# Wionerlol/MultimodalEmotionRecognition

Hardware: AMD Instinct MI355X
Metric: 3s-clip train steps/sec (B=32, xattn fusion) at 1/2/4/8 MI355X (higher is better)
Workload: dtype bf16; 1 GPU; ResNet18 + WavLM-base (frozen) + xattn fusion train step (fwd+bwd+Adam); per_gpu_batch=32, global_batch=32, frames=8, image=112, audio_samples=48000, parallelism=dp1

## Files before the change

### multimodalemotionrecognition_amd/csrc/conv.hip

```cpp
#include "conv_common.h"
#include "mer.h"

MER_CT_BUFFER(mer_ct, 512 * 64)
MER_CT_BUFFER(mer_ctp, 4096 * 8)
#define CT(k) CT_AT(mer_ct_buf, k)
#define CTP(k) CTP_AT(mer_ctp_buf, k)

namespace {

template <bool DGRAD>
__device__ __forceinline__ u32x4 conv_a_chunk(const ConvGeom& g, int n, int oh, int ow, bool rowok, int kk, int tap,
                                              int c, int r, int s) {
  u32x4 v = {0u, 0u, 0u, 0u};
  if (!rowok || kk >= g.Kred) return v;
  int ih, iw;
  if (!DGRAD) {
    ih = oh * g.st - g.pad + r;
    iw = ow * g.st - g.pad + s;
  } else {
    const int th = oh + g.pad - r, tw = ow + g.pad - s;
    if (th < 0 || tw < 0) return v;
    if (g.st == 1) {
      ih = th;
      iw = tw;
// ... 848 lines not shown
        const int kk = k0 + bcl[j];
        const bool ok = bok[j] && kk < Kr;
        const bf16_t* src = !PAR ? pb[j] + kk : (kk >= Kr0 ? pb2[j] + (kk - Kr0) : pb[j] + par_b_off(kk));
        glds16(ok ? src : zero, lb + (w * IB + j) * 512);
      }
      k0 += KS;
    });
  }
  CTP(2);

  auto out_row = [&](int row) -> long {
    if (!PAR) return (long)row;
    const int n = row / (pc.Hc * pc.Wc);
    const int rem = row - n * pc.Hc * pc.Wc;
    const int hh = rem / pc.Wc, ww = rem - hh * pc.Wc;
    return ((long)n * g.OH + 2 * hh + pc.ph) * g.OW + 2 * ww + pc.pw;
  };
  auto red_row = [&]() -> long {
    long row_id = ty;
    if (PAR)
      for (int c2 = 0; c2 < par_cls(); ++c2) {
        const ParClass q = par_class(g, c2);
        row_id += (g.N * q.Hc * q.Wc + BM_ - 1) / BM_;
      }
    return row_id;
  };
  constexpr int EWF = STAGES * BUF / 2 / WAVES;
  const int ct_slot = 10;
  if constexpr (KG > 1) {
    using L = KgLayout<BM_, BN_, WAVES * KG>;
    constexpr int LDR = BN_ + 4;
    constexpr int TM2 = BM_ / L::WM, TN2 = BN_ / L::WN, FM2 = TM2 / 16, FN2 = TN2 / 16;
    using E2 = EpiGeo<FM2, FN2, EWF>;
    const int w2 = t >> 6, wr2 = w2 / L::WN, wc2 = w2 % L::WN;
    constexpr bool PF = DGRAD && E2::NP == 1;
    EpiPre<E2::NP> pre;
    if constexpr (PF)
      conv_epilogue_prefetch<DGRAD, FM2, FN2, L::WM, L::WN, EWF, decltype(out_row), E2::NP, X2>(g, pre, w2, lane, m0,
                                                                                                n0, M, out_row);
    __syncthreads();
    float* const part = reinterpret_cast<float*>(smem_all);
    {
      float* mine = part + kg * BM_ * LDR;
#pragma unroll
      for (int i = 0; i < FM; ++i)
#pragma unroll
        for (int j = 0; j < FN; ++j)
#pragma unroll
          for (int r = 0; r < 4; ++r) mine[(wr * TM + i * 16 + fq * 4 + r) * LDR + wc * TN + j * 16 + fr] = acc[i][j][r];
    }
    lds_barrier();
    f32x4 acc2[FM2][FN2];
#pragma unroll
    for (int i = 0; i < FM2; ++i)
#pragma unroll
      for (int j = 0; j < FN2; ++j)
#pragma unroll
        for (int r = 0; r < 4; ++r) {
          const int e = (wr2 * TM2 + i * 16 + fq * 4 + r) * LDR + wc2 * TN2 + j * 16 + fr;
          float s = part[e];
#pragma unroll
          for (int q = 1; q < KG; ++q) s += part[q * BM_ * LDR + e];
          acc2[i][j][r] = s;
        }
    lds_barrier();
    CTP(3);
    if constexpr (PF)
      conv_epilogue_vec<DGRAD, FM2, FN2, L::WM, L::WN, EWF, decltype(out_row), decltype(pre), false, X2>(
          g, acc2, reinterpret_cast<float*>(smem_all), w2, lane, m0, n0, M, g.bnr_red ? red_row() : 0l, ty, out_row,
          &pre, ct_slot);
    else
      conv_epilogue_vec<DGRAD, FM2, FN2, L::WM, L::WN, EWF, decltype(out_row), EpiNone, false, X2>(
          g, acc2, reinterpret_cast<float*>(smem_all), w2, lane, m0, n0, M, (DGRAD && g.bnr_red) ? red_row() : 0l, ty,
          out_row, static_cast<const EpiNone*>(nullptr), ct_slot);
    CTP(4);
    return;
  }
  if (g.vec) {
    using E1 = EpiGeo<FM, FN, EWF>;
    if constexpr (DGRAD && E1::NP == 1) {
      EpiPre<E1::NP> pre;
      conv_epilogue_prefetch<DGRAD, FM, FN, WM, WN, EWF, decltype(out_row), E1::NP, X2>(g, pre, w, lane, m0, n0, M,
                                                                                         out_row);
      __syncthreads();
      CTP(3);
      conv_epilogue_vec<DGRAD, FM, FN, WM, WN, EWF, decltype(out_row), decltype(pre), false, X2>(
          g, acc, reinterpret_cast<float*>(smem), w, lane, m0, n0, M, g.bnr_red ? red_row() : 0l, ty, out_row, &pre,
          ct_slot);
    } else {
      __syncthreads();
      CTP(3);
      conv_epilogue_vec<DGRAD, FM, FN, WM, WN, EWF, decltype(out_row), EpiNone, false, X2>(
          g, acc, reinterpret_cast<float*>(smem), w, lane, m0, n0, M, (DGRAD && g.bnr_red) ? red_row() : 0l, ty,
          out_row, static_cast<const EpiNone*>(nullptr), ct_slot);
    }
    CTP(4);
    return;
  } else {
  __syncthreads();
#pragma unroll
  for (int i = 0; i < FM; ++i)
#pragma unroll
    for (int r = 0; r < 4; ++r) {
      const int row = m0 + wr * TM + i * 16 + fq * 4 + r;
      if (row >= M) continue;
      const long orow = out_row(row) * g.ldy;
#pragma unroll
      for (int j = 0; j < FN; ++j) {
        const int col = n0 + wc * TN + j * 16 + fr;
        if (col >= g.Ncols) continue;
        float v = acc[i][j][r];
        if (g.R_) {
          const long ri = orow + col;
          if (!g.Rmask || bf2f(g.Rmask[ri]) > 0.f) v += bf2f(g.R_[ri]);
        }
        const bf16_t h = f2bf(v);
        g.Y[orow + col] = h;
        acc[i][j][r] = bf2f(h);
      }
    }
  if (DGRAD && g.bnr_red) {
    float ps[FN][3];
#pragma unroll
    for (int j = 0; j < FN; ++j) {
      const int col = n0 + wc * TN + j * 16 + fr;
      const bool cok = col < g.Ncols;
      const float mu = cok ? g.bnr_ms[2 * col] : 0.f, rs = cok ? g.bnr_ms[2 * col + 1] : 0.f;
      const float mu2 = (cok && g.bnr_x2) ? g.bnr_ms2[2 * col] : 0.f;
      const float rs2 = (cok && g.bnr_x2) ? g.bnr_ms2[2 * col + 1] : 0.f;
      float s1 = 0.f, s2 = 0.f, s3 = 0.f;
#pragma unroll
      for (int i = 0; i < FM; ++i)
#pragma unroll
        for (int r = 0; r < 4; ++r) {
          const int row = m0 + wr * TM + i * 16 + fq * 4 + r;
          if (row < M && cok) {
            const long e = out_row(row) * g.ldy + col;
            const float gv = bf2f(g.bnr_mask[e]) > 0.f ? acc[i][j][r] : 0.f;
            s1 += gv;
            s2 += gv * (bf2f(g.bnr_x[e]) - mu) * rs;
            if (g.bnr_x2) s3 += gv * (bf2f(g.bnr_x2[e]) - mu2) * rs2;
          }
        }
#pragma unroll
      for (int o = 16; o < 64; o <<= 1) {
        s1 += __shfl_xor(s1, o, 64);
        s2 += __shfl_xor(s2, o, 64);
        s3 += __shfl_xor(s3, o, 64);
      }
      ps[j][0] = s1;
      ps[j][1] = s2;
      ps[j][2] = s3;
    }
    float* red = reinterpret_cast<float*>(smem);
    __syncthreads();
    if (wr > 0 && fq == 0)
#pragma unroll
      for (int j = 0; j < FN; ++j)
#pragma unroll
        for (int q = 0; q < 3; ++q) red[((wr * WN + wc) * FN * 16 + j * 16 + fr) * 3 + q] = ps[j][q];
    __syncthreads();
    if (wr == 0 && fq == 0) {
      long row_id = ty;
      if (PAR)
        for (int c2 = 0; c2 < par_cls(); ++c2) {
          const ParClass q = par_class(g, c2);
          row_id += (g.N * q.Hc * q.Wc + BM_ - 1) / BM_;
        }
      const long slab = row_id * g.Ncols * 2;
#pragma unroll
      for (int j = 0; j < FN; ++j) {
        const int col = n0 + wc * TN + j * 16 + fr;
        float t0 = ps[j][0], t1 = ps[j][1], t2 = ps[j][2];
#pragma unroll
        for (int q = 1; q < WM; ++q) {
          const float* o = red + ((q * WN + wc) * FN * 16 + j * 16 + fr) * 3;
          t0 += o[0];
          t1 += o[1];
          t2 += o[2];
        }
        if (col < g.Ncols) {
          g.bnr_red[slab + 2 * col] = t0;
          g.bnr_red[slab + 2 * col + 1] = t1;
          if (g.bnr_red2) {
            g.bnr_red2[slab + 2 * col] = t0;
            g.bnr_red2[slab + 2 * col + 1] = t2;
          }
        }
      }
    }
  }
  }
  if (g.stats) conv_tile_stats<FM, FN, WM, WN>(g, acc, reinterpret_cast<float*>(smem), w, lane, m0, n0, M, ty);
}

template <int BM_, int BN_, int WM_ = 2, int WN_ = 2, int STAGES_ = 2, int KS_ = 64, int KG_ = 1>
struct Tile {
  static constexpr int BM = BM_, BN = BN_, WM = WM_, WN = WN_, STAGES = STAGES_, KS = KS_, KG = KG_;
};

enum ConvFamily { kConvNone, kConvHalo, kConvReg, kConvPipe };

struct ConvPlan {
  int err;
  ConvFamily family;
  int halo;
  int variant;
  bool par;
  int BM, BN, WM, WN, STAGES, KS, KG;
  bool x2, fast;
  size_t lds;
  unsigned grid_x, grid_y;
  int rows;
};

template <bool DGRAD, bool PAR, class T>
int launch_conv_pipe_t(ConvGeom& g, const ConvPlan& p, hipStream_t st) {
  if (T::BM != p.BM || T::BN != p.BN || T::WM != p.WM || T::WN != p.WN || T::STAGES != p.STAGES || T::KS != p.KS ||
      T::KG != p.KG)
    return (int)hipErrorInvalidConfiguration;
  auto launch = [&](void (*kern)(ConvGeom)) -> int {
    if (hipFuncSetAttribute(reinterpret_cast<const void*>(kern), hipFuncAttributeMaxDynamicSharedMemorySize,
                            (int)p.lds) != hipSuccess)
      return (int)hipErrorInvalidConfiguration;
    hipLaunchKernelGGL(kern, dim3(p.grid_x, p.grid_y), dim3(64 * T::WM * T::WN * T::KG), p.lds, st, g);
    return (int)hipGetLastError();
  };
  if constexpr (DGRAD && !PAR) {
    if (!p.x2)
      return p.fast ? launch(&conv_pipe_kernel<DGRAD, PAR, T::BM, T::BN, T::WM, T::WN, T::STAGES, T::KS, false, T::KG,
                                               true>)
                    : launch(&conv_pipe_kernel<DGRAD, PAR, T::BM, T::BN, T::WM, T::WN, T::STAGES, T::KS, false, T::KG,
                                               false>);
  }
  return p.fast
             ? launch(&conv_pipe_kernel<DGRAD, PAR, T::BM, T::BN, T::WM, T::WN, T::STAGES, T::KS, true, T::KG, true>)
             : launch(&conv_pipe_kernel<DGRAD, PAR, T::BM, T::BN, T::WM, T::WN, T::STAGES, T::KS, true, T::KG, false>);
}

inline int conv_bn(const ConvGeom& g) { return g.Ncols <= 64 ? 64 : 128; }
inline bool conv_small_m(const ConvGeom& g, bool par) {
  const long M = (long)g.N * g.OH * g.OW / (par ? 4 : 1);
  const int bn = conv_bn(g);
  return ((M + 127) / 128) * ((g.Ncols + bn - 1) / bn) * (par ? 4 : 1) < 384;
}

template <bool DGRAD, bool PAR, class F>
int conv_pipe_tile(const ConvGeom& g, int variant, F&& f) {
  const int bn = conv_bn(g);
  const bool small_m = conv_small_m(g, PAR);
  if (variant == 7) {
    if (bn == 64) return PAR ? f(Tile<64, 64, 2, 2, 2, 64, 2>{}) : f(Tile<64, 64, 2, 2, 3, 64, 2>{});
    return PAR ? f(Tile<64, 128, 2, 4, 2, 64, 2>{}) : f(Tile<64, 128, 2, 4, 3, 64, 2>{});
  }
  if (variant == 3 && !small_m) {
    if constexpr (DGRAD) {
      return f(Tile<256, 64, 4, 2>{});
    } else {
      if (bn == 64) return f(Tile<256, 64, 4, 2>{});
      return f(Tile<256, 128, 4, 4>{});
    }
  }
  if (variant == 5) {
    if (bn == 64) return small_m ? f(Tile<64, 64, 2, 2, 4, 32>{}) : f(Tile<128, 64, 2, 2, 4, 32>{});
    return small_m ? f(Tile<64, 128, 2, 2, 4, 32>{}) : f(Tile<128, 128, 2, 4, 4, 32>{});
  }
  if (variant == 4) {
    if (bn == 64) return small_m ? f(Tile<64, 64, 2, 2, 3>{}) : f(Tile<128, 64, 4, 2, 3>{});
    return small_m ? f(Tile<64, 128, 2, 4, 3>{}) : f(Tile<128, 128, 2, 4, 3>{});
  }
  if (variant >= 2) {
    if (bn == 64)
      return small_m ? (PAR ? f(Tile<64, 64, 2, 2>{}) : f(Tile<64, 64, 2, 2, 3>{})) : f(Tile<128, 64, 4, 2>{});
    return small_m ? (PAR ? f(Tile<64, 128, 2, 4>{}) : f(Tile<64, 128, 2, 4, 3>{})) : f(Tile<128, 128, 2, 4>{});
  }
  if (bn == 64) return small_m ? f(Tile<64, 64>{}) : f(Tile<128, 64>{});
  return small_m ? f(Tile<64, 128>{}) : f(Tile<128, 128>{});
}

template <bool DGRAD>
int launch_conv(ConvGeom& g, const ConvPlan& p, hipStream_t st) {
  auto launch = [&](void (*kern)(ConvGeom)) -> int {
    hipLaunchKernelGGL(kern, dim3(p.grid_x), dim3(256), 0, st, g);
    return (int)hipGetLastError();
  };
  if (p.BN == 64) return p.BM == 64 ? launch(&conv_kernel<DGRAD, 64, 64>) : launch(&conv_kernel<DGRAD, 128, 64>);
  return p.BM == 64 ? launch(&conv_kernel<DGRAD, 64, 128>) : launch(&conv_kernel<DGRAD, 128, 128>);
}

namespace halo {
constexpr int BM = 128;
template <int C_, int R_, int PAD_, int W_, int IHX_>
struct Geo {
  static constexpr int C = C_, R = R_, PAD = PAD_, W = W_, IHX = IHX_;
  static constexpr int KRED = R * R * C, WCH = KRED / 8;
  static constexpr int CPP = C / 8;
  static constexpr int HW = W + R - 1;
  static constexpr int ROWS = (W + BM - 2) / W + 1 + (R - 1) + IHX;
  static constexpr int CH = (ROWS * HW * CPP + 63) / 64 * 64;
  static constexpr int ELEMS = CH * 8;
  static constexpr int LDS_ELEMS = 64 * KRED + 2 * ELEMS + C;
  static constexpr int KSTEPS = KRED / 32;
  static constexpr int HSHIFT = CPP == 8 ? 1 : 3;
  static_assert(CPP == 8 || CPP == 2, "halo layouts for 16 or 64 channels");
  static_assert(WCH % 16 == 0 || WCH % 16 == 8, "weight-row swizzle");
};
template <int WCH>
__device__ __forceinline__ int wchunk(int n, int c) {
  return WCH % 16 == 0 ? ((c & ~15) | ((c & 15) ^ (n & 15))) : ((c & ~7) | ((c & 7) ^ ((n >> 1) & 7)));
}
}

template <bool DGRAD, class GE, int WM, int WN, int OCC, bool X2 = true>
__global__ __launch_bounds__(64 * WM * WN, OCC) void conv_halo_kernel(ConvGeom g) {
  constexpr int WAVES = WM * WN;
  constexpr int TM = halo::BM / WM, TN = 64 / WN, FM = TM / 16, FN = TN / 16;
  constexpr int HW = GE::HW, CPP = GE::CPP, C = GE::C, R = GE::R, PAD = GE::PAD, W_ = GE::W;
  extern __shared__ __attribute__((aligned(16))) bf16_t smem[];
  bf16_t* const wlds = smem;
  bf16_t* const hbuf = smem + 64 * GE::KRED;
  bf16_t* const zpix = hbuf + 2 * GE::ELEMS;
  const int t = threadIdx.x, lane = t & 63, w = t >> 6;
  const int wr = w / WN, wc = w % WN, fr = lane & 15, fq = lane >> 4;
  const int OH = g.OH, IH = g.IH, IW = g.IW, M = g.N * g.OH * W_, in_rows = g.N * g.IH;
  const int ntiles = (M + halo::BM - 1) / halo::BM;
  const bf16_t* zero = reinterpret_cast<const bf16_t*>(mer_conv_zero16);
  int tile = blockIdx.x;
  CT(0);
  auto in_row0 = [&](int m) {
    const int go = m / W_, n = go / OH;
    return n * IH + (go - n * OH) - PAD;
  };
  auto stage_halo = [&](bf16_t* hb, int tl) {
    const int base = in_row0(tl * halo::BM);
    for (int j = w; j < GE::CH / 64; j += WAVES) {
      const int L = j * 64 + lane;
      const int hp = L / CPP, c = (L % CPP) ^ ((hp >> GE::HSHIFT) & (CPP - 1));
      const int hr = hp / HW, x = hp - hr * HW - PAD, gr = base + hr;
      const bool ok = hr < GE::ROWS && gr >= 0 && gr < in_rows && x >= 0 && x < IW;
      glds16(ok ? g.X + ((long)gr * IW + x) * C + c * 8 : zero, hb + j * 512);
    }
  };
  for (int j = w; j < GE::WCH; j += WAVES) {
    const int L = j * 64 + lane;
    const int n = L / GE::WCH, pc = L - n * GE::WCH;
    glds16(g.Wt + (long)n * GE::KRED + halo::wchunk<GE::WCH>(n, pc) * 8, wlds + j * 512);
  }
  stage_halo(hbuf, tile);
  if (t < CPP) *reinterpret_cast<u32x4*>(zpix + t * 8) = u32x4{0u, 0u, 0u, 0u};
  wait_vmcnt<0>();
  __syncthreads();
  CT(1);

  EpiAcc<FN> eacc;
  eacc.zero();
  for (int cur = 0, it = 0; tile < ntiles; tile += gridDim.x, cur ^= 1, ++it) {
    bf16_t* const hb = hbuf + cur * GE::ELEMS;
    if (tile + (int)gridDim.x < ntiles) stage_halo(hbuf + (cur ^ 1) * GE::ELEMS, tile + gridDim.x);
    CT(it < 11 ? 2 + 5 * it : 63);
    const int m0 = tile * halo::BM, base = in_row0(m0);
    const auto out_row = [](int row) { return (long)row; };
    constexpr int EWF = GE::ELEMS / 2 / WAVES;
    EpiPre<EpiGeo<FM, FN, EWF>::NP> pre;
    if constexpr (DGRAD)
      conv_epilogue_prefetch<DGRAD, FM, FN, WM, WN, EWF, decltype(out_row), EpiGeo<FM, FN, EWF>::NP, X2>(
          g, pre, w, lane, m0, 0, M, out_row);
    int hpb[FM], yv[FM];
#pragma unroll
    for (int i = 0; i < FM; ++i) {
      int m = m0 + wr * TM + i * 16 + fr;
      m = m < M ? m : M - 1;
      const int go = m / W_, x = m - go * W_, n = go / OH, y = go - n * OH;
      yv[i] = y - PAD;
      hpb[i] = (n * IH + y - PAD - base) * HW + x;
    }
    f32x4 acc[FM][FN];
#pragma unroll
    for (int i = 0; i < FM; ++i)
#pragma unroll
      for (int j = 0; j < FN; ++j) acc[i][j] = f32x4{0.f, 0.f, 0.f, 0.f};
    bf16x8 af[2][FM], bfr[2][FN];
    auto frags = [&](int u, bf16x8 (&a)[FM], bf16x8 (&b)[FN]) {
      const int kk = u * 32 + fq * 8;
      const int tap = kk / C, c = (kk % C) / 8;
      const int r = tap / R, s = tap - R * (tap / R);
      const int hr = DGRAD ? R - 1 - r : r, hs = DGRAD ? R - 1 - s : s;
#pragma unroll
      for (int i = 0; i < FM; ++i) {
        const int hp = hpb[i] + hr * HW + hs;
        const bool ok = (unsigned)(yv[i] + hr) < (unsigned)IH;
        a[i] = *reinterpret_cast<const bf16x8*>(
            ok ? hb + hp * C + ((c ^ ((hp >> GE::HSHIFT) & (CPP - 1))) << 3) : zpix);
      }
#pragma unroll
      for (int j = 0; j < FN; ++j) {
        const int n = wc * TN + j * 16 + fr, cb = u * 4 + fq;
        b[j] = *reinterpret_cast<const bf16x8*>(wlds + n * GE::KRED + (halo::wchunk<GE::WCH>(n, cb) << 3));
      }
    };
    frags(0, af[0], bfr[0]);
#pragma unroll
    for (int u = 0; u < GE::KSTEPS; ++u) {
      if (u + 1 < GE::KSTEPS) frags(u + 1, af[(u + 1) & 1], bfr[(u + 1) & 1]);
#pragma unroll
      for (int i = 0; i < FM; ++i)
#pragma unroll
        for (int j = 0; j < FN; ++j)
          acc[i][j] = __builtin_amdgcn_mfma_f32_16x16x32_bf16(af[u & 1][i], bfr[u & 1][j], acc[i][j], 0, 0, 0);
    }
    CT(it < 11 ? 3 + 5 * it : 63);
    wait_vmcnt<0>();
    lds_barrier();
    CT(it < 11 ? 4 + 5 * it : 63);
    const int ct_slot = it == 1 ? 60 : -1;
    if constexpr (DGRAD)
      conv_epilogue_vec<DGRAD, FM, FN, WM, WN, EWF, decltype(out_row), decltype(pre), true, X2, EpiAcc<FN>>(
          g, acc, reinterpret_cast<float*>(hb), w, lane, m0, 0, M, (long)tile, (long)tile, out_row, &pre, ct_slot,
          &eacc);
    else
      conv_epilogue_vec<DGRAD, FM, FN, WM, WN, EWF, decltype(out_row), EpiNone, true, true, EpiAcc<FN>>(
          g, acc, reinterpret_cast<float*>(hb), w, lane, m0, 0, M, (long)tile, (long)tile, out_row,
          static_cast<const EpiNone*>(nullptr), ct_slot, &eacc);
    CT(it < 11 ? 5 + 5 * it : 63);
    lds_barrier();
    CT(it < 11 ? 6 + 5 * it : 63);
  }
  conv_epilogue_acc_finish<DGRAD, FM, FN, WM, WN, GE::ELEMS / 2 / WAVES, X2>(g, eacc, reinterpret_cast<float*>(hbuf), w,
                                                                          lane, 0, (long)blockIdx.x);
}

using HaloL1 = halo::Geo<64, 3, 1, 28, 0>;
using HaloStem = halo::Geo<16, 4, 0, 56, 3>;

int halo_kind(const ConvGeom& g, bool dgrad) {
  if (g.st != 1 || g.Ncols != 64 || g.ldy != 64 || !g.vec || g.X2 != nullptr ||
      ((((uintptr_t)g.X) | ((uintptr_t)g.Wt)) & 15) != 0)
    return 0;
  if (g.R == 3 && g.S == 3 && g.pad == 1 && g.IC == 64 && g.IW == 28 && g.OW == 28 && g.IH == g.OH && g.Kred == 576)
    return 1;
  if (!dgrad && g.R == 4 && g.S == 4 && g.pad == 0 && g.IC == 16 && g.IW == 59 && g.OW == 56 && g.IH == 59 &&
      g.OH == 56 && g.Kred == 256)
    return 2;
  return 0;
}

template <bool DGRAD, class GE, int OCC, bool X2 = true>
int launch_halo_t(ConvGeom& g, const ConvPlan& p, hipStream_t st) {
  constexpr int WM = 4, WN = 2;
  const size_t lds = GE::LDS_ELEMS * sizeof(bf16_t);
  static_assert(GE::LDS_ELEMS * 2 * OCC <= 160 * 1024, "LDS per CU");
  if (hipFuncSetAttribute(reinterpret_cast<const void*>(&conv_halo_kernel<DGRAD, GE, WM, WN, OCC, X2>),
                          hipFuncAttributeMaxDynamicSharedMemorySize, (int)lds) != hipSuccess)
    return (int)hipErrorInvalidConfiguration;
  hipLaunchKernelGGL((conv_halo_kernel<DGRAD, GE, WM, WN, OCC, X2>), dim3(p.grid_x), dim3(64 * WM * WN), lds, st, g);
  return (int)hipGetLastError();
}

constexpr int halo_occ(int kind) { return kind == 1 ? 1 : 2; }

template <bool DGRAD>
int launch_conv_halo(ConvGeom& g, const ConvPlan& p, hipStream_t st) {
  if constexpr (DGRAD)
    if (p.halo == 1 && !p.x2) return launch_halo_t<DGRAD, HaloL1, halo_occ(1), false>(g, p, st);
  if (p.halo == 1) return launch_halo_t<DGRAD, HaloL1, halo_occ(1)>(g, p, st);
  if constexpr (!DGRAD) return launch_halo_t<false, HaloStem, halo_occ(2)>(g, p, st);
  return (int)hipErrorInvalidValue;
}

int conv_default_variant(const ConvGeom& g, int fallback) {
  if (!g.vec || g.Kred < 8 * CBK) return fallback;
  const long M = (long)g.N * g.OH * g.OW;
  const long nt = (g.Ncols + (g.Ncols <= 64 ? 63 : 127)) / (g.Ncols <= 64 ? 64 : 128);
  if (((M + 63) / 64) * nt <= cu_count()) return 7;
  return fallback;
}

template <class F>
int conv_pipe_tile_of(const ConvGeom& g, bool dgrad, bool par, int variant, F&& f) {
  if (!dgrad) return conv_pipe_tile<false, false>(g, variant, f);
  return par ? conv_pipe_tile<true, true>(g, variant, f) : conv_pipe_tile<true, false>(g, variant, f);
}

ConvPlan conv_plan(const ConvGeom& g, bool dgrad, int variant) {
  ConvPlan p{};
  const long M = (long)g.N * g.OH * g.OW;
  const long nx = (g.Ncols + conv_bn(g) - 1) / conv_bn(g);
  p.grid_y = 1;
  p.x2 = true;
  if (variant == -1 || variant == 6) {
    if (const int hk = halo_kind(g, dgrad)) {
      const long ntiles = (M + halo::BM - 1) / halo::BM, slots = (long)halo_occ(hk) * cu_count();
      p.family = kConvHalo;
      p.halo = hk;
      p.variant = 6;
      p.BM = halo::BM; p.BN = 64; p.WM = 4; p.WN = 2;
      p.x2 = !(dgrad && hk == 1 && !g.bnr_x2);
      p.grid_x = (unsigned)(ntiles < slots ? ntiles : slots);
      p.rows = (int)p.grid_x;
      return p;
    }
    if (variant == 6) {
      p.err = (int)hipErrorInvalidValue;
      return p;
    }
    variant = dgrad ? (g.Ncols <= 64 ? 5 : 2) : 2;
    if (!dgrad || g.st == 1) variant = conv_default_variant(g, variant);
  }
  p.variant = variant;
  if (variant == 0 || (dgrad && g.st > 2)) {
    p.family = kConvReg;
    p.BM = conv_small_m(g, false) ? 64 : 128;
    p.BN = conv_bn(g);
    p.WM = p.WN = 2;
    p.rows = (int)((M + p.BM - 1) / p.BM);
    p.grid_x = (unsigned)(nx * p.rows);
    return p;
  }
  p.family = kConvPipe;
  p.par = dgrad && g.st == 2;
  conv_pipe_tile_of(g, dgrad, p.par, variant, [&](auto t) {
    using T = decltype(t);
    p.BM = T::BM; p.BN = T::BN; p.WM = T::WM; p.WN = T::WN; p.STAGES = T::STAGES; p.KS = T::KS; p.KG = T::KG;
    return 0;
  });
  if (p.KG > 1 && !g.vec) p.err = (int)hipErrorInvalidValue;
  const size_t ring = (size_t)p.KG * p.STAGES * (p.BM + p.BN) * p.KS * sizeof(bf16_t);
  const size_t kgred = p.KG > 1 ? (size_t)p.KG * p.BM * (p.BN + 4) * sizeof(float) : 0;
  p.lds = ring > kgred ? ring : kgred;
  p.x2 = !(dgrad && !p.par && !g.bnr_x2);
  p.fast = p.par ? (g.IC % p.KS == 0 && (!g.X2 || g.K2 % p.KS == 0) && ((g.R + 1) / 2) * ((g.S + 1) / 2) <= 32)
                 : (g.IC % p.KS == 0 && g.R * g.S <= 32 && (!dgrad || g.st == 1));
  const long nbn = (g.Ncols + p.BN - 1) / p.BN;
  if (!p.par) {
    p.rows = (int)((M + p.BM - 1) / p.BM);
    p.grid_x = (unsigned)(p.rows * nbn);
    return p;
  }
  p.grid_y = 4;
  for (int cls = 0; cls < 4; ++cls) {
    const int ph = cls >> 1, pw = cls & 1;
    const long Mc = (long)g.N * ((g.OH - ph + 1) >> 1) * ((g.OW - pw + 1) >> 1);
    p.rows += (int)((Mc + p.BM - 1) / p.BM);
    if (cls == 0) p.grid_x = (unsigned)((Mc + p.BM - 1) / p.BM * nbn);
  }
  return p;
}

template <bool DGRAD>
int launch_conv_plan(ConvGeom& g, const ConvPlan& p, hipStream_t st) {
  if (p.err != (int)hipSuccess) return p.err;
  if (p.family == kConvHalo) return launch_conv_halo<DGRAD>(g, p, st);
  if (p.family == kConvReg) return launch_conv<DGRAD>(g, p, st);
  if constexpr (DGRAD)
    if (p.par)
      return conv_pipe_tile<true, true>(g, p.variant,
                                        [&](auto t) { return launch_conv_pipe_t<true, true, decltype(t)>(g, p, st); });
  return conv_pipe_tile<DGRAD, false>(g, p.variant,
                                      [&](auto t) { return launch_conv_pipe_t<DGRAD, false, decltype(t)>(g, p, st); });
}

int conv_plan_rows(const ConvGeom& g, bool dgrad, int variant) {
  const ConvPlan p = conv_plan(g, dgrad, variant);
  if (p.family == kConvHalo || (variant == -1 && p.family == kConvPipe)) return p.rows;
  return (int)(((long)g.N * g.OH * g.OW + 63) / 64 + (dgrad ? 4 : 0));
}

ConvGeom fwd_geom(int N, int H, int W, int C, int K, int R, int S, int stride, int pad, const void* x,
                  const void* w_packed, void* y, float* stats) {
  ConvGeom g{};
  g.N = N; g.IH = H; g.IW = W; g.IC = C;
  g.OH = (H + 2 * pad - R) / stride + 1; g.OW = (W + 2 * pad - S) / stride + 1;
  g.R = R; g.S = S; g.st = stride; g.pad = pad;
  g.Ncols = K; g.Kred = R * S * C;
  g.X = (const bf16_t*)x; g.Wt = (const bf16_t*)w_packed; g.Y = (bf16_t*)y; g.ldy = K; g.stats = stats;
  g.vec = conv_vec_ok(g);
  return g;
}

ConvGeom dgrad_geom(int N, int H, int W, int C, int K, int R, int S, int stride, int pad, const void* dy,
                    const void* wt_packed, const void* ds_dy) {
  ConvGeom g{};
  g.N = N; g.OH = H; g.OW = W;
  g.IH = (H + 2 * pad - R) / stride + 1; g.IW = (W + 2 * pad - S) / stride + 1; g.IC = K;
  g.R = R; g.S = S; g.st = stride; g.pad = pad;
  g.Ncols = C; g.Kred = R * S * K;
  g.X = (const bf16_t*)dy; g.Wt = (const bf16_t*)wt_packed; g.ldy = C; g.stats = nullptr;
  g.X2 = (const bf16_t*)ds_dy;
  g.vec = conv_vec_ok(g);
  return g;
}

}

MER_API int mer_conv_fwd(int N, int H, int W, int C, int K, int R, int S, int stride, int pad, const void* x,
                         const void* w_packed, void* y, float* stats, void* stream) {
  return mer_conv_fwd_ex(N, H, W, C, K, R, S, stride, pad, x, w_packed, y, stats, -1, stream);
}

MER_API int mer_conv_fwd_rows(int N, int H, int W, int C, int K, int R, int S, int stride, int pad, const void* x,
                              const void* w_packed, int variant) {
  if (N <= 0 || C % 8 || variant < -1 || variant > 7) return -(int)hipErrorInvalidValue;
  return conv_plan_rows(fwd_geom(N, H, W, C, K, R, S, stride, pad, x, w_packed, nullptr, nullptr), false, variant);
}

MER_API int mer_conv_dgrad_rows(int N, int H, int W, int C, int K, int R, int S, int stride, int pad, const void* dy,
                                const void* wt_packed, const void* ds_dy, int variant) {
  if (N <= 0 || K % 8 || C % 8 || variant < -1 || variant > 7) return -(int)hipErrorInvalidValue;
  return conv_plan_rows(dgrad_geom(N, H, W, C, K, R, S, stride, pad, dy, wt_packed, ds_dy), true, variant);
}

MER_API int mer_conv_fwd_ex(int N, int H, int W, int C, int K, int R, int S, int stride, int pad, const void* x,
                            const void* w_packed, void* y, float* stats, int variant, void* stream) {
  if (C % 8 || variant < -1 || variant > 7) return (int)hipErrorInvalidValue;
  ConvGeom g = fwd_geom(N, H, W, C, K, R, S, stride, pad, x, w_packed, y, stats);
  return launch_conv_plan<false>(g, conv_plan(g, false, variant), (hipStream_t)stream);
}

MER_API int mer_conv_dgrad(int N, int H, int W, int C, int K, int R, int S, int stride, int pad, const void* dy,
                           const void* wt_packed, void* dx, const void* residual, const void* residual_mask,
                           void* stream) {
  return mer_conv_dgrad_ex(N, H, W, C, K, R, S, stride, pad, dy, wt_packed, dx, residual, residual_mask, -1, stream);
}

MER_API int mer_conv_dgrad_ex(int N, int H, int W, int C, int K, int R, int S, int stride, int pad, const void* dy,
                              const void* wt_packed, void* dx, const void* residual, const void* residual_mask,
                              int variant, void* stream) {
  return mer_conv_dgrad_bnr(N, H, W, C, K, R, S, stride, pad, dy, wt_packed, dx, residual, residual_mask, nullptr,
                            nullptr, nullptr, nullptr, nullptr, nullptr, nullptr, variant, stream);
}

MER_API int mer_conv_dgrad_bnr(int N, int H, int W, int C, int K, int R, int S, int stride, int pad, const void* dy,
                               const void* wt_packed, void* dx, const void* residual, const void* residual_mask,
                               const void* bn_mask, const void* bn_x, const float* bn_ms, float* bn_red,
                               const void* bn_x2, const float* bn_ms2, float* bn_red2, int variant, void* stream) {
  return mer_conv_dgrad_ds(N, H, W, C, K, R, S, stride, pad, dy, wt_packed, dx, residual, residual_mask, bn_mask, bn_x,
                           bn_ms, bn_red, bn_x2, bn_ms2, bn_red2, nullptr, nullptr, 0, variant, stream);
}

MER_API int mer_conv_dgrad_ds(int N, int H, int W, int C, int K, int R, int S, int stride, int pad, const void* dy,
                              const void* wt_packed, void* dx, const void* residual, const void* residual_mask,
                              const void* bn_mask, const void* bn_x, const float* bn_ms, float* bn_red,
                              const void* bn_x2, const float* bn_ms2, float* bn_red2, const void* ds_dy,
                              const void* ds_wt_packed, int ds_K, int variant, void* stream) {
  if (K % 8 || C % 8 || variant < -1 || variant > 7) return (int)hipErrorInvalidValue;
  if (ds_dy && (stride != 2 || R != 3 || S != 3 || pad != 1 || !ds_wt_packed || ds_K <= 0 || ds_K % 64 || K % 64 ||
                variant == 0))
    return (int)hipErrorInvalidValue;
  if (bn_red && (!bn_mask || !bn_x || !bn_ms || (bn_x2 && (!bn_ms2 || !bn_red2)))) return (int)hipErrorInvalidValue;
  if (bn_red && (variant == 0 || stride > 2)) return (int)hipErrorInvalidValue;
  ConvGeom g = dgrad_geom(N, H, W, C, K, R, S, stride, pad, dy, wt_packed, ds_dy);
  g.Y = (bf16_t*)dx;
  g.R_ = (const bf16_t*)residual; g.Rmask = (const bf16_t*)residual_mask;
  g.bnr_mask = (const bf16_t*)bn_mask; g.bnr_x = (const bf16_t*)bn_x; g.bnr_ms = bn_ms; g.bnr_red = bn_red;
  g.bnr_x2 = (const bf16_t*)bn_x2; g.bnr_ms2 = bn_ms2; g.bnr_red2 = bn_red2;
  g.Wt2 = (const bf16_t*)ds_wt_packed; g.K2 = ds_dy ? ds_K : 0;
  return launch_conv_plan<true>(g, conv_plan(g, true, variant), (hipStream_t)stream);
}
```

Measured before the change: 216.5 steps/s.

## Precompute halo conv LDS addresses and schedule MFMA/ds_read interleave

The halo conv kernel now computes per-lane staging offsets and LDS fragment base addresses once, then advances tile coordinates incrementally instead of doing divides every tile and every k-step. Inner-loop fragment loads become raw LDS pointers with constant immediate offsets, with the zero-padding row handled by address substitution. Explicit sched_group_barriers interleave ds_reads with MFMAs. This cuts VALU address arithmetic in the hot loop, at the cost of more live registers and fragile offset-range assumptions guarded by static_asserts.

```diff
diff --git a/multimodalemotionrecognition_amd/csrc/conv.hip b/multimodalemotionrecognition_amd/csrc/conv.hip
--- a/multimodalemotionrecognition_amd/csrc/conv.hip
+++ b/multimodalemotionrecognition_amd/csrc/conv.hip
@@ -1174,9 +1174,17 @@
   static constexpr int LDS_ELEMS = 64 * KRED + 2 * ELEMS + C;
   static constexpr int KSTEPS = KRED / 32;
   static constexpr int HSHIFT = CPP == 8 ? 1 : 3;
+  static constexpr int ROWB = HW * C * 2;
+  static constexpr bool row_in_frame(int hr) { return hr >= PAD && hr - PAD <= IHX; }
   static_assert(CPP == 8 || CPP == 2, "halo layouts for 16 or 64 channels");
   static_assert(WCH % 16 == 0 || WCH % 16 == 8, "weight-row swizzle");
+  static_assert((R - 1) * ROWB + 16 <= 65536 && 16 * KRED * 2 + KRED * 2 <= 65536, "ds_read offset: is 16-bit");
+  static_assert(W >= 16 && ROWS * HW * C < 65536, "one row carry per 16 pixels; stage_halo packs a source offset in 16 bits");
 };
+template <class GE>
+__device__ __forceinline__ int hswz(int col) {
+  return (col >> GE::HSHIFT) & (GE::CPP - 1);
+}
 template <int WCH>
 __device__ __forceinline__ int wchunk(int n, int c) {
   return WCH % 16 == 0 ? ((c & ~15) | ((c & 15) ^ (n & 15))) : ((c & ~7) | ((c & 7) ^ ((n >> 1) & 7)));
@@ -1199,18 +1207,47 @@
   const bf16_t* zero = reinterpret_cast<const bf16_t*>(mer_conv_zero16);
   int tile = blockIdx.x;
   CT(0);
-  auto in_row0 = [&](int m) {
+  auto split = [&](int m, int& gr, int& y, int& x) {
     const int go = m / W_, n = go / OH;
-    return n * IH + (go - n * OH) - PAD;
+    x = m - go * W_;
+    y = go - n * OH;
+    gr = n * IH + y;
   };
-  auto stage_halo = [&](bf16_t* hb, int tl) {
-    const int base = in_row0(tl * halo::BM);
-    for (int j = w; j < GE::CH / 64; j += WAVES) {
-      const int L = j * 64 + lane;
-      const int hp = L / CPP, c = (L % CPP) ^ ((hp >> GE::HSHIFT) & (CPP - 1));
-      const int hr = hp / HW, x = hp - hr * HW - PAD, gr = base + hr;
-      const bool ok = hr < GE::ROWS && gr >= 0 && gr < in_rows && x >= 0 && x < IW;
-      glds16(ok ? g.X + ((long)gr * IW + x) * C + c * 8 : zero, hb + j * 512);
+  auto advance = [&](int& gr, int& y, int& x, int dgr, int dy, int dx) {
+    x += dx;
+    const bool cx = x >= W_;
+    x -= cx ? W_ : 0;
+    y += dy + (cx ? 1 : 0);
+    const bool cy = y >= OH;
+    y -= cy ? OH : 0;
+    gr += dgr + (cx ? 1 : 0) + (cy ? IH - OH : 0);
+  };
+  int sgr, sy, sx;
+  split((int)gridDim.x * halo::BM, sgr, sy, sx);
+  int tgr, ty, tx;
+  split(tile * halo::BM, tgr, ty, tx);
+  int lgr, ly, lx;
+  split(tile * halo::BM + wr * TM + fr, lgr, ly, lx);
+  constexpr int NPC = GE::CH / 64, NK = (NPC + WAVES - 1) / WAVES;
+  int spk[NK];
+#pragma unroll
+  for (int k = 0; k < NK; ++k) {
+    const int L = (w + k * WAVES) * 64 + lane;
+    const int hp = L / CPP, pc = L % CPP;
+    const int hr = hp / HW, col = hp - hr * HW, x = col - PAD;
+    const bool ok = hr < GE::ROWS && x >= 0 && x < IW;
+    spk[k] = ok ? (hr << 16) | ((hr * IW + x) * C + ((pc ^ halo::hswz<GE>(col)) << 3)) : -1;
+  }
+  auto stage_halo = [&](bf16_t* hb, int gr0) {
+    const int base = gr0 - PAD;
+    const bf16_t* xb = g.X + (long)base * (IW * C);
+#pragma unroll
+    for (int k = 0; k < NK; ++k) {
+      const int j = w + k * WAVES;
+      if (j < NPC) {
+        const bool ok = spk[k] >= 0 && (unsigned)(base + (spk[k] >> 16)) < (unsigned)in_rows;
+        glds16(ok ? xb + (spk[k] & 0xffff) : zero, hb + j * 512);
+      }
     }
   };
   for (int j = w; j < GE::WCH; j += WAVES) {
@@ -1218,8 +1255,18 @@
     const int n = L / GE::WCH, pc = L - n * GE::WCH;
     glds16(g.Wt + (long)n * GE::KRED + halo::wchunk<GE::WCH>(n, pc) * 8, wlds + j * 512);
   }
-  stage_halo(hbuf, tile);
+  stage_halo(hbuf, tgr);
   if (t < CPP) *reinterpret_cast<u32x4*>(zpix + t * 8) = u32x4{0u, 0u, 0u, 0u};
+  constexpr int WLOW = GE::WCH % 16 == 0 ? 16 : 8, NWV = WLOW / 4;
+  typedef const bf16x8 __attribute__((address_space(3))) * lds_frag;
+  const unsigned lds0 = (unsigned)reinterpret_cast<uintptr_t>(smem);
+  unsigned wb[NWV];
+#pragma unroll
+  for (int v = 0; v < NWV; ++v) {
+    const int n = wc * TN + fr;
+    wb[v] = lds0 + 2 * (n * GE::KRED + (halo::wchunk<GE::WCH>(n, v * 4 + fq) << 3));
+    asm volatile("" : "+v"(wb[v]));
+  }
   wait_vmcnt<0>();
   __syncthreads();
   CT(1);
@@ -1228,23 +1275,46 @@
   eacc.zero();
   for (int cur = 0, it = 0; tile < ntiles; tile += gridDim.x, cur ^= 1, ++it) {
     bf16_t* const hb = hbuf + cur * GE::ELEMS;
-    if (tile + (int)gridDim.x < ntiles) stage_halo(hbuf + (cur ^ 1) * GE::ELEMS, tile + gridDim.x);
+    const int gr0 = tgr;
+    advance(tgr, ty, tx, sgr, sy, sx);
+    if (tile + (int)gridDim.x < ntiles) stage_halo(hbuf + (cur ^ 1) * GE::ELEMS, tgr);
     CT(it < 11 ? 2 + 5 * it : 63);
-    const int m0 = tile * halo::BM, base = in_row0(m0);
+    const int m0 = tile * halo::BM;
     const auto out_row = [](int row) { return (long)row; };
     constexpr int EWF = GE::ELEMS / 2 / WAVES;
     EpiPre<EpiGeo<FM, FN, EWF>::NP> pre;
     if constexpr (DGRAD)
       conv_epilogue_prefetch<DGRAD, FM, FN, WM, WN, EWF, decltype(out_row), EpiGeo<FM, FN, EWF>::NP, X2>(
           g, pre, w, lane, m0, 0, M, out_row);
-    int hpb[FM], yv[FM];
-#pragma unroll
-    for (int i = 0; i < FM; ++i) {
-      int m = m0 + wr * TM + i * 16 + fr;
-      m = m < M ? m : M - 1;
-      const int go = m / W_, x = m - go * W_, n = go / OH, y = go - n * OH;
-      yv[i] = y - PAD;
-      hpb[i] = (n * IH + y - PAD - base) * HW + x;
+    constexpr int NAV = CPP == 8 ? 2 * R : 2;
+    const unsigned zoff = lds0 + 2 * (64 * GE::KRED + 2 * GE::ELEMS);
+    unsigned ab[FM][NAV];
+    bool rok[FM][R];
+    {
+      int gr = lgr, y = ly, x = lx;
+#pragma unroll
+      for (int i = 0; i < FM; ++i) {
+        if (i > 0) advance(gr, y, x, 0, 0, 16);
+        const int pix = (gr - gr0) * HW + x;
+        const int hoff = 64 * GE::KRED + cur * GE::ELEMS;
+#pragma unroll
+        for (int v = 0; v < NAV; ++v) {
+          int s, c;
+          if constexpr (CPP == 8) {
+            s = v >> 1;
+            c = (v & 1) * 4 + fq;
+          } else {
+            s = 2 * v + (fq >> 1);
+            c = fq & 1;
+          }
+          const int hs = DGRAD ? R - 1 - s : s;
+          ab[i][v] = lds0 + 2 * (hoff + (pix + hs) * C + ((c ^ halo::hswz<GE>(x + hs)) << 3));
+          asm volatile("" : "+v"(ab[i][v]));
+        }
+#pragma unroll
+        for (int hr = 0; hr < R; ++hr) rok[i][hr] = (unsigned)(y - PAD + hr) < (unsigned)IH;
+      }
+      advance(lgr, ly, lx, sgr, sy, sx);
     }
     f32x4 acc[FM][FN];
 #pragma unroll
@@ -1253,24 +1323,22 @@
       for (int j = 0; j < FN; ++j) acc[i][j] = f32x4{0.f, 0.f, 0.f, 0.f};
     bf16x8 af[2][FM], bfr[2][FN];
     auto frags = [&](int u, bf16x8 (&a)[FM], bf16x8 (&b)[FN]) {
-      const int kk = u * 32 + fq * 8;
-      const int tap = kk / C, c = (kk % C) / 8;
-      const int r = tap / R, s = tap - R * (tap / R);
-      const int hr = DGRAD ? R - 1 - r : r, hs = DGRAD ? R - 1 - s : s;
-#pragma unroll
-      for (int i = 0; i < FM; ++i) {
-        const int hp = hpb[i] + hr * HW + hs;
-        const bool ok = (unsigned)(yv[i] + hr) < (unsigned)IH;
-        a[i] = *reinterpret_cast<const bf16x8*>(
-            ok ? hb + hp * C + ((c ^ ((hp >> GE::HSHIFT) & (CPP - 1))) << 3) : zpix);
-      }
-#pragma unroll
-      for (int j = 0; j < FN; ++j) {
-        const int n = wc * TN + j * 16 + fr, cb = u * 4 + fq;
-        b[j] = *reinterpret_cast<const bf16x8*>(wlds + n * GE::KRED + (halo::wchunk<GE::WCH>(n, cb) << 3));
-      }
+      const int r = CPP == 8 ? (u / 2) / R : (2 * u) / R;
+      const int v = CPP == 8 ? ((u / 2) % R) * 2 + (u & 1) : (u & 1);
+      const int hr = DGRAD ? R - 1 - r : r;
+      auto afrag = [&](int i) {
+        const unsigned e = GE::row_in_frame(hr) ? ab[i][v] : (rok[i][hr] ? ab[i][v] : zoff - hr * GE::ROWB);
+        a[i] = *reinterpret_cast<lds_frag>(e + hr * GE::ROWB);
+      };
+      afrag(0);
+#pragma unroll
+      for (int j = 0; j < FN; ++j)
+        b[j] = *reinterpret_cast<lds_frag>(wb[u % NWV] + ((u / NWV) * WLOW * 8 + j * 16 * GE::KRED) * 2);
+#pragma unroll
+      for (int i = 1; i < FM; ++i) afrag(i);
     };
     frags(0, af[0], bfr[0]);
+    __builtin_amdgcn_sched_barrier(0);
 #pragma unroll
     for (int u = 0; u < GE::KSTEPS; ++u) {
       if (u + 1 < GE::KSTEPS) frags(u + 1, af[(u + 1) & 1], bfr[(u + 1) & 1]);
@@ -1279,6 +1347,14 @@
 #pragma unroll
         for (int j = 0; j < FN; ++j)
           acc[i][j] = __builtin_amdgcn_mfma_f32_16x16x32_bf16(af[u & 1][i], bfr[u & 1][j], acc[i][j], 0, 0, 0);
+      static_assert(FM + FN == 4 && FM * FN >= 2, "the step's issue pattern");
+      __builtin_amdgcn_sched_group_barrier(0x002, FM, 0);
+      __builtin_amdgcn_sched_group_barrier(0x008, 1, 0);
+      __builtin_amdgcn_sched_group_barrier(0x100, 2, 0);
+      __builtin_amdgcn_sched_group_barrier(0x008, 1, 0);
+      __builtin_amdgcn_sched_group_barrier(0x100, 2, 0);
+      __builtin_amdgcn_sched_group_barrier(0x008, FM * FN - 2, 0);
+      __builtin_amdgcn_sched_barrier(0);
     }
     CT(it < 11 ? 3 + 5 * it : 63);
     wait_vmcnt<0>();
```

Measured after the change: 216.5 steps/s, median of 3. Within noise of the previous version (+0.0%).
